# refresh-bio/fqsqueezer

Measured on AMD Instinct MI355X. Metric: Mbases/s compressed (DNA stream, SE sorted), higher is better.
Workload: dtype u64; 1 GPU; 1000000x150bp SE, G=7500000 (seed 2+rank), -om s -gs 8 -qm n -im n; workers_T=64, blocks=256, per_gpu=one independent file per GPU

## Files before the change

fqsqueezer_amd/codec.py:

```python
from __future__ import annotations

import ctypes as C
import os
from typing import List, Optional

import numpy as np

_PKG = os.path.dirname(os.path.abspath(__file__))
DEFAULT_LIB = os.path.join(_PKG, "libfqsx.so")

STAT_NAMES = ["gprobe", "gslot", "lprobe", "lslot", "gins", "gins_slot", "siv_words", "ctx_slots",
              "coded", "lins", "mail", "bases", "siv_saved", "dec_refetch"]


class FqsxError(RuntimeError):
    pass


def _load(path: str):
    if not os.path.exists(path):
        raise FqsxError(f"{path} not found: build it with `python -c 'import __graft_entry__ as g; g.build()'` "
                        "(hipcc --offload-arch=gfx950); there is no CPU fallback")
    try:
        import torch
    except ImportError:
        pass
    lib = C.CDLL(path)
    lib.fqsx_dna_create.restype = C.c_int
    lib.fqsx_dna_create.argtypes = [C.c_char_p, C.c_int, C.POINTER(C.c_void_p)]
    if hasattr(lib, "fqsx_dna_create_on_partition"):
        lib.fqsx_dna_create_on_partition.restype = C.c_int
        lib.fqsx_dna_create_on_partition.argtypes = [C.c_char_p, C.c_int, C.c_uint32, C.c_uint32, C.POINTER(C.c_void_p)]
    lib.fqsx_dna_destroy.argtypes = [C.c_void_p]
    lib.fqsx_dna_encode_block.restype = C.c_int
    lib.fqsx_dna_encode_block.argtypes = [C.c_void_p, C.c_void_p, C.c_void_p, C.c_uint32, C.c_uint32,
                                          C.POINTER(C.c_void_p), C.POINTER(C.c_uint64)]
    lib.fqsx_dna_encode_block_dev.restype = C.c_int
    lib.fqsx_dna_encode_block_dev.argtypes = [C.c_void_p, C.c_void_p, C.c_void_p, C.c_void_p, C.c_uint32, C.c_uint32,
                                              C.POINTER(C.c_void_p), C.POINTER(C.c_uint64)]
    lib.fqsx_dna_decode_block.restype = C.c_int
    lib.fqsx_dna_decode_block.argtypes = [C.c_void_p, C.POINTER(C.c_char_p), C.c_void_p, C.c_void_p, C.c_uint32, C.c_uint32, C.c_void_p]
    lib.fqsx_dna_stats.restype = C.c_int
    lib.fqsx_dna_stats.argtypes = [C.c_void_p, C.POINTER(C.c_uint64)]
    if hasattr(lib, "fqsx_dna_capacity"):
        lib.fqsx_dna_capacity.restype = C.c_int
# ... 352 lines not shown
```

fqsqueezer_amd/csrc/fqsx_api.hip:

```cpp
#include "fqsx_kernels.h"
#include "fqsx_qual.h"
#include "fqsx_qdec.h"
#include "../../include/fqsx.h"
#include "fqsx_vm.h"
#include "fqsx_rt.h"
#include <sys/resource.h>

#ifndef FQSX_EMU
#include <dlfcn.h>
#include <rccl/rccl.h>
#endif
#include <algorithm>
#include <cstdio>
#include <cstdlib>
#include <cstring>
#include <string>
#include <vector>

extern "C" const char *fqsx_last_error(void) { return g_err.c_str(); }
extern "C" const char *fqsx_version(void) {
#ifdef FQSX_EMU
  return "fqsx 0.1 (host emulation build - tests only)";
#else
  return "fqsx 0.1 (HIP gfx950)";
#endif
}

FQ_DEV bool phase_skip(const DevCfg &cfg) { return (cfg.err[0] | cfg.err[1]) != 0; }
#define FQSX_INS_THREADS 128
FQ_KERNEL128 void k_insert_phase(DevCfg cfg, u64 nb_slots, u64 ns_slots) {
  FQ_SHARED InsShared sm;
  if (phase_skip(cfg)) return;
#ifndef FQSX_EMU
  if (threadIdx.x == 0) { sm.pf_done = 0; sm.pf_on = blockDim.x > 64 ? 1u : 0u; }
  __syncthreads();
  if (FQ_WAVE_ID == 1) {
    if (FQ_BLOCK < 3 * cfg.T) insert_prefetch_body(cfg, &sm, FQ_BLOCK / 3, FQ_BLOCK % 3);
    return;
  }
#else
  sm.pf_done = 0; sm.pf_on = 0;
#endif
  if (FQ_BLOCK >= 3 * cfg.T) {
    const u64 stride = (u64)(FQ_NBLOCKS - 3 * cfg.T) * FQ_WAVE, first = (u64)(FQ_BLOCK - 3 * cfg.T) * FQ_WAVE + FQ_LANE;
    for (u64 i = first; i < nb_slots; i += stride) cfg.l_b.slots[i] = 0;
    for (u64 i = first; i < ns_slots; i += stride) cfg.l_s.slots[i] = 0;
    for (u64 i = first; i < 2ull * cfg.T; i += stride) cfg.l_s.filled[i] = 0;
    return;
  }
  insert_phase_body(cfg, &sm, FQ_BLOCK / 3, FQ_BLOCK % 3);
  if (cfg.sys_scope) fq_release_system();
}
FQ_KERNEL64 void k_compact_streams(DevCfg cfg, const u64 *lens, u8 *dst) {
  const u32 tid = FQ_BLOCK;
  u64 off = 0;
  for (u32 t = 0; t < tid; ++t) off += lens[t];
  const u64 n = lens[tid] <= cfg.out_cap ? lens[tid] : 0;
  const u8 *src = cfg.out + (u64)tid * cfg.out_cap;
  for (u64 i = FQ_LANE; i < n; i += FQ_WAVE) dst[off + i] = src[i];
}
FQ_KERNEL64 void k_compact_generic(const u8 *out, u64 out_cap, const u64 *lens, u8 *dst) {
  const u32 tid = FQ_BLOCK;
  u64 off = 0;
  for (u32 t = 0; t < tid; ++t) off += lens[t];
  const u64 n = lens[tid] <= out_cap ? lens[tid] : 0;
  const u8 *src = out + (u64)tid * out_cap;
  for (u64 i = FQ_LANE; i < n; i += FQ_WAVE) dst[off + i] = src[i];
}
FQ_KERNEL64 void k_clear_local(DevCfg cfg, u64 nb_slots, u64 ns_slots) {
  if (phase_skip(cfg)) return;
  const u64 stride = (u64)FQ_NBLOCKS * FQ_WAVE, first = (u64)FQ_BLOCK * FQ_WAVE + FQ_LANE;
  for (u64 i = first; i < nb_slots; i += stride) cfg.l_b.slots[i] = 0;
  for (u64 i = first; i < ns_slots; i += stride) cfg.l_s.slots[i] = 0;
  for (u64 i = first; i < 2ull * cfg.T; i += stride) cfg.l_s.filled[i] = 0;
}
FQ_KERNEL64 void k_finish_block(DevCfg cfg, u64 *lens , u64 *end ) {
  if (FQ_LANE == 0) {
    if (FQ_BLOCK == 0) { end[2 * cfg.T] = cfg.err[0]; end[2 * cfg.T + 1] = cfg.err[1]; }
    if (cfg.err[1]) return;
    finish_block_body(cfg, FQ_BLOCK);
    lens[FQ_BLOCK] = cfg.ws[FQ_BLOCK].out_len;
    end[FQ_BLOCK] = cfg.ws[FQ_BLOCK].out_len;
    end[cfg.T + FQ_BLOCK] = cfg.ctx_filled[FQ_BLOCK];
  }
// ... 436 lines not shown
  u32 cur_n_reads, cur_S, cur_gen;
  u64 cur_need_lb, cur_need_ls, cur_need_lpe;
  bool cur_decode;
  u32 shard_rank, shard_world = 1;
  u8 *d_vmap;
  u64 *d_xbuf;
  u64 xbuf_cap;
  u32 *d_cglob;
  u32 *d_colsum;
  u64 siv_before[2];
  fqsx_comm comm;
  bool comm_set, shard_apply_own;
  u64 *d_xrecv[3];
  u64 xrecv_cap[3];
  u64 *d_items, *d_gathered, *d_small;
  u64 items_cap, gathered_cap;
  std::vector<u32> h_cglob;
  u64 sh_phases, sh_collectives, sh_a2a_words, sh_gather_words;
  bool part;
  bool part_fallback;
  u64 vm_gran;
  fqsx_vm::FdMesh mesh;
  struct VmTab {
    u8 *va = nullptr;
    u64 va_bytes = 0, chunk_bytes = 0;
    std::vector<fqsx_vm::Handle> h;
    std::vector<u8> mapped;
    u64 own_bytes = 0;
    u32 own_mod = 0;
    bool live = false;
  } vm_s, vm_b, vm_pk, vm_pv, vm_siv;
  u32 *d_plog_n;
  u32 ins_threads;
  u64 vm_own_bytes;
};

namespace {

#define FQSX_PIN_BYTES (64u * 1024u)
int d2h_small_begin(fqsx_dna *c, const void *d, u64 bytes) { return d2h(c, c->h_pin, d, bytes); }
int d2h_small_end(fqsx_dna *c, void *h, u64 bytes) {
  DEVCHK(dev_sync(c));
  memcpy(h, c->h_pin, bytes);
  return FQSX_OK;
}

#define REHASH_GRID FQ_GRID(2048)

int collect_streams(DevCtx *c, u8 *&d_compact, u64 &compact_cap, u32 T, const u8 *d_out, u64 out_cap, const u64 *d_lens,
                    const std::vector<u64> &lens_host, std::vector<u8> &h_out, const u8 **streams, u64 *lens) {
  int rc;
  void *p = nullptr;
  u64 total = 0;
  for (u32 t = 0; t < T; ++t) total += lens_host[t];
  if (total > compact_cap) {
    dfree(c, d_compact);
    d_compact = nullptr; compact_cap = 0;
    if ((rc = dalloc(c, &p, total + total / 2 + 4096, false))) return rc;
    d_compact = (u8 *)p;
    compact_cap = total + total / 2 + 4096;
  }
  h_out.resize(total ? total : 1);
  if (total) {
    LAUNCH(c, 2, k_compact_generic, T, 64, d_out, out_cap, d_lens, d_compact);
    if ((rc = d2h_sync(c, h_out.data(), d_compact, total))) return rc;
  }
// ... 417 lines not shown
  }
  cfg.bases = d_bases;
  cfg.read_off = d_off;
  if (decode) {
    std::vector<u64> doff(T + 1, 0);
    for (u32 t = 0; t < T; ++t) doff[t + 1] = doff[t] + dec_lens[t];
    u64 max_len = 0;
    for (u32 i = 0; i < n_reads; ++i) max_len = std::max(max_len, h_off[i + 1] - h_off[i]);
    const u64 need_in = doff[T] + 64, need_out = h_off[n_reads] + 64, need_sc = max_len + 64;
    if (need_in > c->din_cap) {
      dfree(c, (void *)cfg.din);
      if ((rc = dalloc(c, &p, need_in + need_in / 4, false))) return rc;
      cfg.din = (const u8 *)p; c->din_cap = need_in + need_in / 4;
    }
    if (need_out > c->dout_cap) {
      dfree(c, cfg.dout);
      if ((rc = dalloc(c, &p, need_out + need_out / 4, false))) return rc;
      cfg.dout = (u8 *)p; c->dout_cap = need_out + need_out / 4;
    }
    if (need_sc > cfg.dcap) {
      dfree(c, cfg.dscratch);
      if ((rc = dalloc(c, &p, (u64)T * 2 * (need_sc + need_sc / 4), false))) return rc;
      cfg.dscratch = (u8 *)p; cfg.dcap = need_sc + need_sc / 4;
    }
    if (!cfg.din_off && (rc = dalloc(c, &p, ((u64)T + 1) * sizeof(u64), false))) return rc;
    if (!cfg.din_off) cfg.din_off = (const u64 *)p;
    std::vector<u8> flat(doff[T] ? doff[T] : 1);
    for (u32 t = 0; t < T; ++t) memcpy(flat.data() + doff[t], dec_streams[t], dec_lens[t]);
    if ((rc = h2d(c, (void *)cfg.din, flat.data(), doff[T]))) return rc;
    if ((rc = h2d(c, (void *)cfg.din_off, doff.data(), (T + 1) * sizeof(u64)))) return rc;
    DEVCHK(dev_sync(c));
  }

  c->cur_n_reads = n_reads; c->cur_S = (u32)S; c->cur_gen = generation;
  c->cur_need_lb = need_lb; c->cur_need_ls = need_ls; c->cur_need_lpe = need_lpe;
  c->cur_decode = decode;
  return FQSX_OK;
}

int clear_local_tables(fqsx_dna *c) {
  const u64 words = (c->cur_need_lb + c->cur_need_ls) * c->T;
  const u32 grid = (u32)std::min<u64>(2048, (words + 4095) / 4096 + 1);
  LAUNCH(c, 2, k_clear_local, grid, 64, c->cfg, c->cur_need_lb * c->T, c->cur_need_ls * c->T);
  return FQSX_OK;
}

int insert_and_clear(fqsx_dna *c) {
  const u64 words = (c->cur_need_lb + c->cur_need_ls) * c->T;
  const u32 cgrid = (u32)std::min<u64>(2048, (words + 4095) / 4096 + 1);
  LAUNCH(c, 1, k_insert_phase, 3 * c->T + cgrid, c->ins_threads, c->cfg, c->cur_need_lb * c->T, c->cur_need_ls * c->T);
  return FQSX_OK;
}
int grow_for_demand(fqsx_dna *c) {
  const u32 T = c->T;
  DevCfg &cfg = c->cfg;
  int rc;
  for (int which = 0; which < 2; ++which) {
    KTab &t = which ? cfg.g_b : cfg.g_s;
    u64 &cap = which ? c->gb_cap : c->gs_cap;
    u64 need = 0;
    for (u32 o = 0; o < T; ++o) need = std::max<u64>(need, (u64)c->h_demand[2 * T + 1 + which * T + o] + c->h_demand[which * T + o]);
    if (tab_over(c, need, cap) && (rc = grow_global(c, t, cap, tab_new_cap(c, need)))) return rc;
  }
  return FQSX_OK;
}
int pe_insert_and_clear(fqsx_dna *c);
int pe_clear_local(fqsx_dna *c);
int block_recover(fqsx_dna *c, u32 seg) {
  const u32 T = c->T;
  int rc;
  if ((rc = d2h_sync(c, c->h_demand.data(), c->d_demand, (4 * T + 1) * sizeof(u32)))) return rc;
  const u64 before = c->gs_cap + c->gb_cap + c->gpe_cap;
  if ((rc = grow_for_demand(c))) return rc;
  if ((rc = dzero(c, c->cfg.err + 1, sizeof(u32)))) return rc;
  if (c->paired) {
    if ((rc = dzero(c, c->cfg.pe_bkt_n, T * sizeof(u32)))) return rc;
    LAUNCH(c, 2, k_pe_demand, T, 64, c->cfg, c->d_demand + 4 * T + 1, 0u);
    std::vector<u32> dem(T), fil(T);
    if ((rc = d2h_sync(c, dem.data(), c->d_demand + 4 * T + 1, T * sizeof(u32)))) return rc;
    if ((rc = d2h_sync(c, fil.data(), c->cfg.g_pe.filled, T * sizeof(u32)))) return rc;
    u64 need = 0;
    for (u32 o = 0; o < T; ++o) need = std::max<u64>(need, (u64)fil[o] + dem[o]);
    if (need * 2 > c->gpe_cap && (rc = grow_gpe(c, pow2_at_least(need * 2 + 2)))) return rc;
  }
  if (c->gs_cap + c->gb_cap + c->gpe_cap == before) { g_err = "phase " + std::to_string(seg) + " posted for growth, but no table needs it"; return FQSX_E_DEVICE; }
  if (c->paired && (rc = pe_insert_and_clear(c))) return rc;
  return insert_and_clear(c);
}
int pe_clear_local(fqsx_dna *c) {
  const u32 T = c->T;
  DevCfg &cfg = c->cfg;
  int rc;
  if ((rc = dzero(c, cfg.l_pe.key, c->cur_need_lpe * T * sizeof(u64)))) return rc;
  if ((rc = dzero(c, cfg.l_pe.val, c->cur_need_lpe * T * sizeof(u64)))) return rc;
  return dzero(c, cfg.l_pe.filled, T * sizeof(u32));
}
int pe_insert_and_clear(fqsx_dna *c) {
  LAUNCH(c, 2, k_pe_insert, c->T, 64, c->cfg);
  return pe_clear_local(c);
}

int block_segment(fqsx_dna *c, u32 seg) {
  const u32 T = c->T, n_reads = c->cur_n_reads;
  const u64 S = c->cur_S, need_lpe = c->cur_need_lpe;
  const bool decode = c->cur_decode;
  DevCfg &cfg = c->cfg;
  int rc;
  {
    if ((rc = launch_segment(c, decode, n_reads, (u32)S, seg))) return rc;
    const u32 part_grid = T * (cfg.mail[0].n_tiles + cfg.mail[1].n_tiles + cfg.mail[2].n_tiles);
    LAUNCH(c, 2, k_part_count, part_grid, 64, cfg);
    LAUNCH(c, 2, k_part_scan, 3 * T, 64, cfg);
    if (!decode) {
      LAUNCH(c, 2, k_part_scatter, part_grid, 64, cfg, seg + 1, c->d_demand);
      if (c->paired) {
        const u32 bgrid = FQ_GRID((u32)std::min<u64>(1024, ((u64)T * cfg.pe_cap + 255) / 256));
        LAUNCH(c, 2, k_pe_bucket_count, bgrid, 256, cfg);
        LAUNCH(c, 2, k_pe_bucket_offsets, 1, 64, cfg, seg + 1);
        LAUNCH(c, 2, k_pe_bucket_scatter, bgrid, 256, cfg);
        LAUNCH(c, 2, k_pe_insert_buckets, T, 64, cfg);
        if ((rc = pe_clear_local(c))) return rc;
      }
      return insert_and_clear(c);
    }
    LAUNCH(c, 2, k_part_dstoff, 3, 64, cfg, c->d_demand, 0u);
    if ((rc = d2h_small_begin(c, c->d_demand, (4 * T + 1) * sizeof(u32)))) return rc;
    LAUNCH(c, 2, k_part_scatter, part_grid, 64, cfg, 0u, (u32 *)nullptr);
    if ((rc = d2h_small_end(c, c->h_demand.data(), (4 * T + 1) * sizeof(u32)))) return rc;
    if (c->h_demand[2 * T]) {
      g_err = "device error " + std::to_string(c->h_demand[2 * T]) + " in encode kernel";
      return FQSX_E_DEVICE;
    }
    if ((rc = grow_for_demand(c))) return rc;
    if (c->paired) {
      LAUNCH(c, 2, k_pe_demand, T, 64, cfg, c->d_demand, 0u);
      if ((rc = d2h_sync(c, c->h_demand.data(), c->d_demand, T * sizeof(u32)))) return rc;
      if ((rc = d2h_sync(c, c->h_filled.data(), cfg.g_pe.filled, T * sizeof(u32)))) return rc;
      u64 need = 0;
      for (u32 o = 0; o < T; ++o) need = std::max<u64>(need, (u64)c->h_filled[o] + c->h_demand[o]);
      if (need * 2 > c->gpe_cap && (rc = grow_gpe(c, pow2_at_least(need * 2 + 2)))) return rc;
      if ((rc = pe_insert_and_clear(c))) return rc;
    }
// ... 73 lines not shown
    seg = posted;
  }
  return rc;
}

int create_impl(fqsx_dna *c, const u8 *h) {
  const u32 T = c->T;
  DevCfg &cfg = c->cfg;
  memset(&cfg, 0, sizeof(cfg));
  cfg.T = T;
  cfg.mode = h[5];
  cfg.prefix = h[10]; cfg.pmer = h[11]; cfg.smer = h[12]; cfg.bmer = h[13];
  cfg.gp = make_geom(cfg.pmer); cfg.gs = make_geom(cfg.smer); cfg.gb = make_geom(cfg.bmer);
  cfg.pmer_mod_shift = 2 * cfg.pmer - 12;
  cfg.T_magic = ((1ull << 32) + T - 1) / T;
  cfg.T_pow2 = (T & (T - 1)) == 0 ? 1u : 0u;
  cfg.dbg = 0;
  if (const char *e = getenv("FQSX_PROTO_DEBUG")) cfg.dbg = (u32)strtoul(e, nullptr, 0);
  cfg.ps_nobytes_n = (2 * cfg.pmer + 7) / 8;
  int rc;
  void *p = nullptr;
  if ((rc = dalloc(c, &p, (1ull << (2 * cfg.pmer)) / 4, true))) return rc;
  cfg.siv = (u64 *)p;
  if ((rc = dalloc(c, &p, 2 * sizeof(u64), true))) return rc;
  cfg.siv_stats = (u64 *)p;
  if ((rc = dalloc(c, &p, ((1ull << (2 * cfg.pmer)) >> FQSX_SIV_BLK_LOG) * 4 * sizeof(u32), true))) return rc;
  cfg.siv_idx = (u32 *)p;
  c->tab_load_pct = 80; c->tab_after_pct = 62;
  if (const char *e = getenv("FQSX_TAB_LOAD_PCT")) c->tab_load_pct = (u32)std::min<u64>(85, std::max<u64>(20, strtoull(e, nullptr, 10)));
  c->tab_small_pct = 40;
  if (const char *e = getenv("FQSX_TAB_AFTER_PCT")) c->tab_small_pct = c->tab_after_pct = (u32)std::min<u64>(c->tab_load_pct - 5, std::max<u64>(10, strtoull(e, nullptr, 10)));
  cfg.tab_load_pct = c->tab_load_pct;
  c->ins_threads = (getenv("FQSX_INS_PREFETCH") && atoi(getenv("FQSX_INS_PREFETCH")) == 0) ? 64u : FQSX_INS_THREADS;
  if (const char *e = getenv("FQSX_WHATIF")) { u32 r = 0, u = 0; if (sscanf(e, "%u,%u", &r, &u) == 2) cfg.whatif = (r << 16) | (u & 0xffffu); }
  c->gs_cap = c->gb_cap = pow2_at_least(std::max<u64>(1024, (1ull << 22) / T));
  if (const char *e = getenv("FQSX_GTAB_INIT")) c->gs_cap = c->gb_cap = pow2_at_least(std::max<u64>(64, strtoull(e, nullptr, 10)));
  if ((rc = ktab_alloc(c, cfg.g_s, T, c->gs_cap, cfg.smer, 12, true))) return rc;
  if ((rc = ktab_alloc(c, cfg.g_b, T, c->gb_cap, cfg.bmer, 6, true))) return rc;
  cfg.g_s.two = cfg.g_b.two = 1;
  c->ls_cap = c->lb_cap = 1024;
  if ((rc = ktab_alloc(c, cfg.l_s, T, c->ls_cap, cfg.smer, 12, false))) return rc;
  if ((rc = ktab_alloc(c, cfg.l_b, T, c->lb_cap, cfg.bmer, 6, false))) return rc;
  if ((rc = dalloc(c, &p, 2 * (u64)T * sizeof(u32), true))) return rc;
  cfg.l_s.filled = (u32 *)p;
  cfg.l_b.filled = (u32 *)p + T;
  c->ctx_cap = 1u << 14;
  if ((rc = dalloc(c, &p, c->ctx_cap * T * sizeof(CtxSlot), true))) return rc;
  cfg.ctx = (CtxSlot *)p;
  cfg.ctx_cap_mask = c->ctx_cap - 1;
  if ((rc = dalloc(c, &p, T * sizeof(u32), true))) return rc;
  cfg.ctx_filled = (u32 *)p;
  {
    std::vector<u16> tpl(SM_OFF_BYTE, 0);
    auto fill = [&](u32 off, u32 entries, u32 stride, u32 n) {
      for (u32 e = 0; e < entries; ++e) {
        for (u32 i = 0; i < n; ++i) tpl[off + e * stride + i] = 1;
        tpl[off + e * stride + n] = (u16)n;
      }
    };
    fill(SM_OFF_FLAGS, 256, SM_FLAGS_N + 1, SM_FLAGS_N);
    fill(SM_OFF_NS, 32, SM_NS_N + 1, SM_NS_N);
    fill(SM_OFF_PSF, 65536, SM_PSF_N + 1, SM_PSF_N);
    fill(SM_OFF_PSNB, 65536, 6, cfg.ps_nobytes_n);
    fill(SM_OFF_NIB, 68, SM_NIB_N + 1, SM_NIB_N);
    tpl.resize(SM_TOTAL_U16, 0);
    fill(SM_OFF_MID, 1, SM_NIB_N + 1, SM_NIB_N);
// ... 706 lines not shown
int fqsx_rccl_comm_rebind(fqsx_comm *m, fqsx_dna *c) {
  if (!m || !m->ctx || !c) { g_err = "bad argument"; return FQSX_E_ARG; }
  ((RcclCtx *)m->ctx)->stream = c->stream;
  return FQSX_OK;
}
int fqsx_rccl_comm_info(fqsx_comm *m, uint32_t out[2]) {
  if (!m || !m->ctx || !out) { g_err = "bad argument"; return FQSX_E_ARG; }
  RcclCtx *x = (RcclCtx *)m->ctx;
  int n = 0, r = 0;
  if (g_rccl.CommCount(x->comm, &n) != ncclSuccess || g_rccl.CommUserRank(x->comm, &r) != ncclSuccess) { g_err = "ncclCommCount / ncclCommUserRank failed"; return FQSX_E_HIP; }
  out[0] = (u32)n; out[1] = (u32)r;
  return FQSX_OK;
}
void fqsx_rccl_comm_destroy(fqsx_comm *m) {
  if (!m || !m->ctx) return;
  RcclCtx *x = (RcclCtx *)m->ctx;
  if (g_rccl.CommDestroy && !x->aborted) (void)g_rccl.CommDestroy(x->comm);
  delete x;
  m->ctx = nullptr;
}
#else
static int no_rccl() { g_err = "the emulation build has no RCCL transport"; return FQSX_E_NO_DEVICE; }
int fqsx_rccl_unique_id(uint8_t *) { return no_rccl(); }
int fqsx_rccl_comm_create(fqsx_dna *, const uint8_t *, uint32_t, uint32_t, fqsx_comm *) { return no_rccl(); }
int fqsx_rccl_comm_rebind(fqsx_comm *, fqsx_dna *) { return no_rccl(); }
int fqsx_rccl_comm_info(fqsx_comm *, uint32_t *) { return no_rccl(); }
void fqsx_rccl_comm_destroy(fqsx_comm *) {}
#endif

int fqsx_dna_stats(fqsx_dna *c, uint64_t out[64]) {
  if (!c || !out) return FQSX_E_ARG;
  DEVCHK(dev_enter(c));
  LAUNCH(c, 2, k_gather_stats, 1, 64, c->cfg, c->d_lens + c->T);
  return d2h_sync(c, out, c->d_lens + c->T, 64 * sizeof(u64));
}

int fqsx_dna_capacity(fqsx_dna *c, uint64_t out[16]) {
  if (!c || !out) return FQSX_E_ARG;
  DEVCHK(dev_enter(c));
  const u32 T = c->T;
  std::vector<u32> f(T);
  int rc;
  for (int i = 0; i < 16; ++i) out[i] = 0;
  if ((rc = d2h_sync(c, f.data(), c->cfg.g_s.filled, T * sizeof(u32)))) return rc;
  for (u32 t = 0; t < T; ++t) out[0] += f[t];
  if ((rc = d2h_sync(c, f.data(), c->cfg.g_b.filled, T * sizeof(u32)))) return rc;
  for (u32 t = 0; t < T; ++t) out[1] += f[t];
  out[2] = c->gs_cap * T;
  out[3] = c->gb_cap * T;
  out[4] = (1ull << (2 * c->cfg.pmer)) / 4;
  out[5] = c->ctx_cap * T;
  if ((rc = d2h_sync(c, f.data(), c->cfg.ctx_filled, T * sizeof(u32)))) return rc;
  for (u32 t = 0; t < T; ++t) out[6] += f[t];
  out[7] = c->dev_bytes;
  out[8] = c->dev_bytes_peak;
  out[9] = c->n_growths;
  if (c->paired) {
    if ((rc = d2h_sync(c, f.data(), c->cfg.g_pe.filled, T * sizeof(u32)))) return rc;
    for (u32 t = 0; t < T; ++t) out[10] += f[t];
    out[11] = c->gpe_cap * T;
  }
  out[12] = sizeof(u64);
  out[13] = (c->vm_s.live ? c->vm_s.own_bytes : c->gs_cap * T * sizeof(u64)) + (c->vm_b.live ? c->vm_b.own_bytes : c->gb_cap * T * sizeof(u64));
  out[15] = c->vm_siv.live ? c->vm_siv.own_bytes : out[4];
  if (c->paired) out[14] = c->vm_pk.live ? c->vm_pk.own_bytes + c->vm_pv.own_bytes : c->gpe_cap * T * 2 * sizeof(u64);
  return FQSX_OK;
}
// ... 781 lines not shown
```

fqsqueezer_amd/csrc/fqsx_dev.h:

```cpp
#pragma once
#include "fqsx_layout.h"

#define FQSX_RR 6u
#define FQSX_SW 4u
#define FQSX_NSC 3u
#define FQSX_SCR FQSX_NSC
#define FQSX_RQ 256u
struct SpecBuf {
  u32 h_read, h_i0, h_n;
  u32 h_epoch;
  u32 h_pub;
  u32 h_fix_lane, h_fix_end;
  u32 h_pq_lo[2];
  u32 h_np, h_nlp;
  u64 h_ns, h_nls;
  u64 sp_sdir[6][FQSX_SPEC];
  u64 sp_src[6][FQSX_SPEC];
  u8 sp_scur[6][FQSX_SPEC];
  u64 sp_key[10][FQSX_SPEC];
  u8 sp_kind[FQSX_SPEC];
  u64 sp_cq[FQSX_SPEC];
  u8 sp_lvz[FQSX_SPEC];
  u8 sp_flag[FQSX_SPEC];
  u8 sp_rsym[FQSX_SPEC];
// ... 60 lines not shown
    u64 kdir[6], krc[6];
    u32 kcur[6];
    u64 s_let[4];
  } sc_req;
  u64 lev_tmp[10];
  u32 fr_idx[64], fr_c0[64], fr_thr[64], fr_vis[64];
  u64 fr_q1[64], fr_q2[64], fr_q3[64];
  u64 fr_same[64];
#ifdef FQSX_EMU
  u32 fr_f[64], fr_c[64], fr_t[64];
#endif
  u8 fr_lvl[64], fr_bad[64];
  u64 pq_key[2][FQSX_PQ];
  u64 ib_pos[64];
  u64 ib_hash[256];
  alignas(8) u32 qm_bits[4][256];
  u32 lq_target[2], lq_done[2], lq_quit;
  u64 cq_key[10][FQSX_CQ];
  u8 cq_kind[FQSX_CQ];
  u8 cq_rsym[FQSX_CQ];
  u32 cq_tail, cq_head, cq_done;
  u32 rq_f[FQSX_RQ], rq_c[FQSX_RQ], rq_t[FQSX_RQ];
  u64 rq_m[FQSX_RQ];
  u32 rq_tail, rq_head, rq_done;
  u32 wg_stop;
};
#ifndef FQSX_EMU
static_assert(sizeof(WgShared) <= 160u * 1024u, "WgShared must fit the 160 KB of LDS of a gfx950 CU");
#endif
struct InsShared {
  u32 mt[4][624];
  u32 mt_idx[4];
  u32 pf_done, pf_on;
  u64 ib_pos[64];
  u64 ib_hash[256];
  u64 bk_key[64];
  u64 pe_bk[3][64];
};
struct EncArgs {
  DevCfg cfg;
  u32 n_reads, S, seg, pad;
};
#ifndef FQSX_EMU
__shared__ WgShared fq_wg_lds;
FQ_DEV WgShared *fq_wg() { return &fq_wg_lds; }
typedef const __attribute__((address_space(4))) EncArgs *FqArgsP;
FQ_DEV FqArgsP fq_kernarg() { return (FqArgsP)__builtin_amdgcn_kernarg_segment_ptr(); }
FQ_DEV const EncArgs *fq_args(FqArgsP a) {
  const unsigned long v = (unsigned long)a;
  const u32 lo = __builtin_amdgcn_readfirstlane((u32)v), hi = __builtin_amdgcn_readfirstlane((u32)(v >> 32));
  return (const EncArgs *)(FqArgsP)(((unsigned long)hi << 32) | lo);
}
#else
typedef const EncArgs *FqArgsP;
FQ_DEV WgShared *fq_wg() { static thread_local WgShared s; return &s; }
FQ_DEV const EncArgs *fq_args(FqArgsP a) { return a; }
#endif
enum { SX_VALID = 1, SX_LB = 2, SX_S = 4, SX_LS = 8, SX_UNC = 16 ,
       SX_HITS = SX_LB | SX_S | SX_LS | SX_UNC };
enum { SCQ_FROM_HEAD = 1 , SCQ_REVERSED = 2  };
enum { SK_NONE = 0, SK_RANK = 1, SK_LETTER = 2, SK_RANK_PENDING = 3, SK_LETTER_PENDING = 4, SK_RAW = 5, SK_KIND_MASK = 7,
       SK_RESET = 8  };
enum { PV_B = 1, PV_S = 2, PV_P = 4, PV_PHID = 8, PV_PCAND = 16 };

struct C4 { u32 c[4]; };
struct Kmer { u64 dir, rc; u32 cur; };
// ... 518 lines not shown
FQ_DEV void batch_hit_mask(Wk &w, u32 n, u64 mask[4]) {
  WgShared *sm = w.sm;
  mask[0] = mask[1] = mask[2] = mask[3] = 0;
#if FQ_WAVE > 1
  for (u32 r = 0; r * 64 < n; ++r) {
    u32 q = r * 64 + FQ_LANE;
    bool hit = q < n && (sm->bk_res[q][0] | sm->bk_res[q][1] | sm->bk_res[q][2] | sm->bk_res[q][3]) != 0;
    mask[r] = wave_ballot(hit);
  }
#else
  for (u32 q = 0; q < n; ++q)
    if (sm->bk_res[q][0] | sm->bk_res[q][1] | sm->bk_res[q][2] | sm->bk_res[q][3]) mask[q >> 6] |= 1ull << (q & 63);
#endif
}
FQ_DEV void batch_count(Wk &w, const KTab &t, u32 n) {
  WgShared *sm = w.sm;
  u64 ns = 0;
  FQ_SYNC();
  for (u32 i = FQ_LANE; i < n; i += FQ_WAVE) {
    u64 key = sm->bk_key[i];
    sm->bk_res[i][0] = tab_count(t, sb_owner(w.cfg, key), key, ns);
  }
  FQ_SYNC();
  w.st[ST_GPROBE] += n;
  w.st[ST_GSLOT] += wave_sum64(ns);
}

template <class SM>
FQ_DEV void insert_batch(const DevCfg &cfg, SM *sm, const KTab &t, u32 sub, const u64 *keys, u32 n, u32 rng, const Cinc &ci,
                         u64 &nslots, u32 &err);
template <class SM>
FQ_DEV void insert_batch_k(const DevCfg &cfg, SM *sm, const KTab &t, u32 sub, u64 mykey, u32 n, u32 rng, const Cinc &ci,
                           u64 &nslots, u32 &err);
template <class SM, bool EXT_PF = false>
FQ_DEV void insert_keys(const DevCfg &cfg, SM *sm, const KTab &t, u32 sub, const u64 *keys, u32 n, u32 rng, const Cinc &ci,
                        u64 &nslots, u32 &err) {
#if FQ_WAVE > 1
  if constexpr (EXT_PF) {
    u64 nextk = FQ_LANE < n ? keys[FQ_LANE] : 0;
    for (u32 o = 0; o < n && !err; o += FQ_WAVE) {
      const u64 k = nextk;
      if (o + FQ_WAVE + FQ_LANE < n) nextk = keys[o + FQ_WAVE + FQ_LANE];
      insert_batch_k(cfg, sm, t, sub, k, n - o < FQ_WAVE ? n - o : FQ_WAVE, rng, ci, nslots, err);
      lds_store_rel(&sm->pf_done, o / FQ_WAVE + 1);
    }
    return;
  }
  const u64 *s = t.slots + (u64)sub * t.stride;
  u64 nextk = FQ_LANE < n ? keys[FQ_LANE] : 0;
  for (u32 o = 0; o < n && !err; o += FQ_WAVE) {
    const u64 k = nextk;
    u64 touch = 0;
    if (o + FQ_WAVE + FQ_LANE < n) {
      nextk = keys[o + FQ_WAVE + FQ_LANE];
      const TabHome th = tab_home(t, nextk >> (64 - 2 * t.k));
      touch = touch_load(&s[(u64)th.a * FQSX_BKT]) ^ touch_load(&s[(u64)th.b * FQSX_BKT]);
    }
    insert_batch_k(cfg, sm, t, sub, k, n - o < FQ_WAVE ? n - o : FQ_WAVE, rng, ci, nslots, err);
    keep_live(touch);
  }
#else
  for (u32 j = 0; j < n && !err; ++j) insert_batch(cfg, sm, t, sub, keys + j, 1, rng, ci, nslots, err);
#endif
}
FQ_DEV u32 lq_done_now(Wk &w, u32 qi) { return w.lqh ? lds_load_acq(&w.sm->lq_done[qi]) : w.la[qi ? MAIL_S : MAIL_B]; }
FQ_DEV void lq_publish(Wk &w, bool force = false) {
// ... 3424 lines not shown
  TM_TRACE_VAL(cfg, tid, launch, 12, w.tm[TM_RRWAIT]); TM_TRACE_VAL(cfg, tid, launch, 13, w.tm[TM_SPEC]);
  TM_TRACE_VAL(cfg, tid, launch, 14, w.tm[CN_GENERIC]); TM_TRACE_VAL(cfg, tid, launch, 15, w.tm[TM_LQ]);
#ifdef FQSX_TIMING
  {
    const u32 xs[16] = {TM_SLOW, TM_SPRE, TM_ROUGH, TM_FINDC, TM_POST, TM_KEYS, TM_READ_HEAD, TM_CQWAIT, TX_QMM, TX_QRUN, TX_PROLOG, TX_CHUNKQ, TX_FLUSH, TM_TOTAL, TX_G_EARLY, TX_OWNSPEC};
    for (u32 x = 0; x < 16; ++x) TM_TRACE_VAL(cfg, tid, launch, 16 + x, w.tm[xs[x]]);
  }
#endif
  if (!piped) {
    for (u32 i = 0; i < ST_N; ++i) ws->stat[i] += w.st[i];
    for (u32 i = 0; i < FQSX_TM_SLOTS && i < 48; ++i) ws->stat[16 + i] += w.tm[i];
  } else if (FQ_LANE == 0) {
    for (u32 i = 0; i < ST_N; ++i) if (w.st[i]) atomic_add64(&ws->stat[i], w.st[i]);
#ifdef FQSX_TIMING
    for (u32 i = 0; i < FQSX_TM_SLOTS && i < 48; ++i) if (w.tm[i]) atomic_add64(&ws->stat[16 + i], w.tm[i]);
#endif
  }
  FQ_SYNC();
  mt_copy((u64 *)&ws->mt[0][0], (const u64 *)&sm->mt[0][0]);
  for (u32 g = FQ_LANE; g < 4; g += FQ_WAVE) ws->mt_idx[g] = sm->mt_idx[g];
  for (u32 k = 0; k < 3; ++k) cfg.mail[k].n[tid] = w.mn[k];
  if (paired) cfg.pe_n[tid] = w.pe_n;
  if (w.err) *cfg.err = w.err;
}

template <class SM>
FQ_DEV void insert_batch(const DevCfg &cfg, SM *sm, const KTab &t, u32 tid, const u64 *keys, u32 n, u32 rng, const Cinc &ci,
                         u64 &nslots, u32 &err) {
  insert_batch_k(cfg, sm, t, tid, FQ_LANE < n ? keys[FQ_LANE] : 0, n, rng, ci, nslots, err);
}
template <class SM>
FQ_DEV void insert_batch_k(const DevCfg &cfg, SM *sm, const KTab &t, u32 tid, u64 mykey, u32 n, u32 rng, const Cinc &ci,
                           u64 &nslots, u32 &err) {
  (void)cfg;
#ifdef FQSX_TIMING
  u64 ib_t[4] = {0, 0, 0, 0}, ib_rounds = 0;
#define IB_MARK(i) do { const u64 now_ = fq_clock(); ib_t[i] += now_ - ib_c; ib_c = now_; } while (0)
  u64 ib_c = fq_clock();
#else
#define IB_MARK(i) ((void)0)
#endif
  u64 *s = t.slots + (u64)tid * t.stride;
  const u64 cm = (1ull << t.cbits) - 1ull;
  const u32 lane = FQ_LANE;
  const u64 v = lane < n ? mykey >> (64 - 2 * t.k) : 0;
  u32 filled = t.filled[tid];
  for (u32 done = 0; done < n;) {
    u64 pos = 0, item = 0;
    bool act = lane >= done && lane < n, found = false;
    if (act) {
      const TabLoc L = t.two ? tab_locate(t, s, v) : tab_locate1(t, s, v);
      pos = L.pos; item = L.item; nslots += L.ns;
      found = item != 0;
    }
    IB_MARK(0);
    u32 lim = n;
#if FQ_WAVE > 1
    FQ_SYNC();
    sm->ib_pos[lane] = act ? pos : ~0ull;
    for (u32 i = lane; i < 256; i += FQ_WAVE) sm->ib_hash[i] = 0;
    FQ_SYNC();
    const u32 hb = (((u32)pos ^ (u32)(pos >> 32)) * 0x9E3779B1u) >> 24;
    if (act) lds_or64(&sm->ib_hash[hb], 1ull << lane);
    FQ_SYNC();
    bool clash = false;
    if (act) {
      u64 cand = sm->ib_hash[hb] & ((1ull << lane) - 1ull);
      while (cand && !clash) {
        const u32 j = ctz64(cand);
        cand &= cand - 1ull;
        clash = sm->ib_pos[j] == pos;
      }
    }
    const u64 cl = wave_ballot(clash);
    if (cl) lim = ctz64(cl);
    act = act && lane < lim;
#else
    lim = done + 1;
#endif
    IB_MARK(1);
    const u32 n_new = popc64(wave_ballot(act && !found));
    if ((u64)(filled + n_new) * 10 >= t.nb * FQSX_BKT * 9) { err = FQSX_ERR_GTAB_FULL; return; }
    const u32 cnt = (u32)(item & cm);
    const bool draw = act && found && cnt > ci.thr && cnt < ci.maxv;
    const u64 dm = wave_ballot(draw);
    u32 r = 0;
    if (dm) {
      const u32 my = popc64(dm & ((1ull << lane) - 1ull)), total = popc64(dm);
      u32 idx = sm->mt_idx[rng];
      const u32 avail = idx >= 624 ? 0 : 624 - idx;
      if (draw && my < avail) r = mt_temper(sm->mt[rng][idx + my]);
      if (total > avail) {
        mt_twist(sm->mt[rng]);
        if (draw && my >= avail) r = mt_temper(sm->mt[rng][my - avail]);
        idx = total - avail;
      } else
        idx += total;
      FQ_SYNC();
      if (lane == 0) sm->mt_idx[rng] = idx;
      FQ_SYNC();
    }
    if (act) {
      if (!found) s[pos] = (v << t.cbits) | 1ull;
      else if (cnt <= ci.thr) { if (cnt < (u32)cm) s[pos] = item + 1; }
      else if (draw && (r % (ci.mult * (cnt - ci.thr)) == 0)) s[pos] = item + 1;
    }
    filled += n_new;
    done = lim;
    if (lane == 0 && done >= n) t.filled[tid] = filled;
    IB_MARK(2);
    FQ_SYNC_MEM();
    IB_MARK(3);
#ifdef FQSX_TIMING
    ++ib_rounds;
#endif
  }
#ifdef FQSX_TIMING
  if (rng < 2 && lane == 0) {
    for (u32 i = 0; i < 4; ++i) atomic_add64(&cfg.ws[tid].stat[16 + 40 + i], ib_t[i]);
    atomic_add64(&cfg.ws[tid].stat[16 + 44], ib_rounds);
// ... 64 lines not shown
    (void)cnt; (void)ld;
    if (e < hi) lds_or64(&gm[d], 1ull << FQ_LANE);
    FQ_SYNC();
    const u64 mine = e < hi ? gm[d] : 0;
    const u32 rank = popc64(mine & ((1ull << FQ_LANE) - 1ull));
    const u32 later = (mine >> FQ_LANE) >> 1 ? 1u : 0u;
    u32 cur = e < hi ? cursor[d] : 0;
    FQ_SYNC();
    if (e < hi) {
      m.sorted[cur + rank] = x;
      if (later == 0) { cursor[d] = cur + rank + 1; gm[d] = 0; }
    }
    FQ_SYNC();
#else
    ld[FQ_LANE] = d;
    FQ_SYNC();
    u32 rank = 0, later = 0;
    for (u32 q = 0; q < cnt; ++q) {
      u32 dq = ld[q];
      rank += (q < FQ_LANE && dq == d) ? 1u : 0u;
      later += (q > FQ_LANE && dq == d) ? 1u : 0u;
    }
    u32 cur = e < hi ? cursor[d] : 0;
    FQ_SYNC();
    if (e < hi) {
      m.sorted[cur + rank] = x;
      if (later == 0) cursor[d] = cur + rank + 1;
    }
    FQ_SYNC();
#endif
  }
}

FQ_DEV void siv_idx_move(const DevCfg &cfg, u64 idx, u32 from, u32 to) {
  u32 *e = cfg.siv_idx + 4 * (idx >> FQSX_SIV_BLK_LOG);
#ifndef FQSX_EMU
  if (from) atomicSub(&e[from], 1u);
  atomicAdd(&e[to], 1u);
#else
  if (from) e[from] -= 1;
  e[to] += 1;
#endif
}
#ifndef FQSX_PF_AHEAD
#define FQSX_PF_AHEAD 4
#endif
#if FQ_WAVE > 1
template <class SM>
FQ_DEV void insert_prefetch_body(const DevCfg &cfg, SM *sm, u32 tid, u32 kind) {
  if (kind == MAIL_P) return;
  const Mail &m = cfg.mail[kind];
  const u32 lo = m.dst_off[tid], hi = m.dst_off[tid + 1], n = hi - lo;
  const KTab &t = kind == MAIL_S ? cfg.g_s : cfg.g_b;
  const u64 *s = t.slots + (u64)tid * t.stride, *keys = m.sorted + lo;
  u64 acc = 0;
  for (u32 o = 0; o < n; o += FQ_WAVE) {
    u32 spins = 0;
    while ((i32)(o / FQ_WAVE - lds_load_acq(&sm->pf_done)) > (i32)FQSX_PF_AHEAD) {
      fq_sleep();
      if (++spins > (1u << 18)) { keep_live(acc); return; }
    }
    if (o + FQ_LANE < n) {
      const TabHome th = tab_home(t, keys[o + FQ_LANE] >> (64 - 2 * t.k));
      acc ^= touch_load(&s[(u64)th.a * FQSX_BKT]) ^ touch_load(&s[(u64)th.b * FQSX_BKT]);
    }
  }
  keep_live(acc);
}
#endif
template <class SM>
FQ_DEV void insert_phase_body(const DevCfg &cfg, SM *sm, u32 tid, u32 kind) {
  WState *ws = cfg.ws + tid;
  const Mail &m = cfg.mail[kind];
  const u32 lo = m.dst_off[tid], hi = m.dst_off[tid + 1];
  if (kind == MAIL_P) {
    u64 nf = 0, nu = 0;
    for (u32 e = lo + FQ_LANE; e < hi; e += FQ_WAVE) {
      u64 idx = m.sorted[e];
      u64 *wp = cfg.siv + (idx >> 5);
      u32 sh = 2 * (u32)(idx & 31);
      u64 old = *wp;
      for (;;) {
        u64 f = (old >> sh) & 3;
        if (f == 3) break;
        u64 seen = atomic_cas64(wp, old, old + (1ull << sh));
        if (seen == old) {
          nf += f == 0;
          siv_idx_move(cfg, idx, (u32)f, (u32)f + 1);
          if (cfg.siv_part) {
#ifndef FQSX_EMU
            const u32 at = atomicAdd(cfg.p_log_n, 1u);
#else
            const u32 at = (*cfg.p_log_n)++;
#endif
            cfg.p_log[at] = (idx << 4) | (f << 2) | (f + 1);
          }
          break;
        }
        old = seen;
      }
      ++nu;
    }
    nf = wave_sum64(nf);
    nu = wave_sum64(nu);
    if (FQ_LANE == 0) {
#ifndef FQSX_EMU
      atomicAdd((unsigned long long *)&cfg.siv_stats[1], (unsigned long long)nf);
      atomicAdd((unsigned long long *)&cfg.siv_stats[0], (unsigned long long)(nu + ws->hidden_updates));
#else
      cfg.siv_stats[1] += nf;
      cfg.siv_stats[0] += nu + ws->hidden_updates;
#endif
      ws->hidden_updates = 0;
      ws->stat[ST_SIV_WORDS] += hi - lo;
    }
    return;
  }
  const KTab &t = kind == MAIL_S ? cfg.g_s : cfg.g_b;
  const u32 rng = kind == MAIL_S ? RNG_S : RNG_B;
  const Cinc ci = kind == MAIL_S ? CINC_S : CINC_B;
  u32 err = 0;
  u64 n_slots = 0;
  FQ_SYNC();
  for (u32 i = FQ_LANE; i < 624; i += FQ_WAVE) sm->mt[rng][i] = ws->mt[rng][i];
  if (FQ_LANE == 0) sm->mt_idx[rng] = ws->mt_idx[rng];
  FQ_SYNC();
  if (sm->pf_on) insert_keys<SM, true>(cfg, sm, t, tid, m.sorted + lo, hi - lo, rng, ci, n_slots, err);
  else insert_keys(cfg, sm, t, tid, m.sorted + lo, hi - lo, rng, ci, n_slots, err);
  FQ_SYNC();
  for (u32 i = FQ_LANE; i < 624; i += FQ_WAVE) ws->mt[rng][i] = sm->mt[rng][i];
  n_slots = wave_sum64(n_slots);
  if (FQ_LANE == 0) {
    ws->mt_idx[rng] = sm->mt_idx[rng];
#ifndef FQSX_EMU
    atomicAdd((unsigned long long *)&ws->stat[ST_GINS], (unsigned long long)(hi - lo));
    atomicAdd((unsigned long long *)&ws->stat[ST_GINS_SLOT], (unsigned long long)n_slots);
#else
    ws->stat[ST_GINS] += hi - lo;
    ws->stat[ST_GINS_SLOT] += n_slots;
#endif
  }
  if (err) *cfg.err = err;
}

FQ_DEV void finish_block_body(const DevCfg &cfg, u32 tid) {
  WState *ws = cfg.ws + tid;
  u64 low = ws->rc_low, len = ws->out_len;
  u8 *out = cfg.out + (u64)tid * cfg.out_cap;
  for (int i = 0; i < 8; ++i) {
    if (len < cfg.out_cap) out[len] = (u8)(low >> 56); else *cfg.err = FQSX_ERR_OUT_OVERFLOW;
    ++len;
    low <<= 8;
  }
  ws->rc_low = low;
  ws->out_len = len;
}
```

Baseline: 109.8 Mbases/s.

## Fuse mail partition, demand check and global insert into one phase-tail kernel

Adds a k_phase_tail kernel that replaces the per-phase sequence of partition count/scan/scatter and insert launches with a single launch. Each owner workgroup gathers its mailbox keys directly into LDS using multiple waves, writes demand and the growth flag itself, then inserts with a companion prefetch wave. It also loads the Mersenne-Twister state lazily, only when a random draw is actually needed. The goal is to cut kernel-launch and global sort/scatter traffic per phase, at the cost of a done-stamp recovery protocol, more complex control flow, and a key-count limit above which the old split path is used.

Measured after the change: 110.2 Mbases/s (median of 6 runs). Within noise of the previous version (+0.4%).

```diff
diff --git a/fqsqueezer_amd/codec.py b/fqsqueezer_amd/codec.py
--- a/fqsqueezer_amd/codec.py
+++ b/fqsqueezer_amd/codec.py
@@ -10,7 +10,7 @@
 DEFAULT_LIB = os.path.join(_PKG, "libfqsx.so")
 
 STAT_NAMES = ["gprobe", "gslot", "lprobe", "lslot", "gins", "gins_slot", "siv_words", "ctx_slots",
-              "coded", "lins", "mail", "bases", "siv_saved", "dec_refetch"]
+              "coded", "lins", "mail", "bases", "siv_saved", "dec_refetch", "phases_fused", "phases_split"]
 
 
 class FqsxError(RuntimeError):
diff --git a/fqsqueezer_amd/csrc/fqsx_api.hip b/fqsqueezer_amd/csrc/fqsx_api.hip
--- a/fqsqueezer_amd/csrc/fqsx_api.hip
+++ b/fqsqueezer_amd/csrc/fqsx_api.hip
@@ -50,6 +50,102 @@
   }
   insert_phase_body(cfg, &sm, FQ_BLOCK / 3, FQ_BLOCK % 3);
   if (cfg.sys_scope) fq_release_system();
+}
+#define FQSX_TAIL_THREADS (64u * FQSX_TAIL_WAVES)
+#define FQSX_TAIL_TOTAL_MAX 65536u
+FQ_KERNEL512 void k_phase_tail(DevCfg cfg, u64 nb_slots, u64 ns_slots, u32 seg1, u32 *demand , u32 *done ,
+                               u32 stamp, u32 stage, u32 recover) {
+  FQ_SHARED TailShared sm;
+  const u32 T = cfg.T, wave = FQ_WAVE_ID;
+#ifndef FQSX_EMU
+  const u32 nw = blockDim.x >> 6, tix = threadIdx.x;
+#else
+  const u32 nw = 1, tix = 0;
+#endif
+  const bool owner_wg = FQ_BLOCK < 3 * T;
+  const u32 d = FQ_BLOCK / 3, kind = FQ_BLOCK % 3;
+  u32 e0 = 0, e1 = 0, dn = 0, fl = 0;
+  if (tix == 0) {
+    e0 = cfg.err[0]; e1 = cfg.err[1];
+    if (owner_wg) {
+      dn = done[kind * T + d];
+      if (kind != MAIL_P) fl = (kind == MAIL_S ? cfg.g_s : cfg.g_b).filled[d];
+    }
+  }
+  if (owner_wg) {
+    for (u32 i = tix; i < T; i += nw * FQ_WAVE) sm.n_src[i] = cfg.mail[kind].n[i];
+    for (u32 i = tix; i < 256; i += nw * FQ_WAVE) sm.vm[i] = cfg.vmap[i];
+  }
+  if (tix == 0) {
+    bool go = !(e0 || (e1 && e1 != seg1));
+    if (go && owner_wg && recover && dn == stamp) go = false;
+    sm.go = go ? 1u : 0u;
+    sm.filled = fl;
+    sm.ins.pf_done = 0; sm.ins.pf_on = 0; sm.ins.mt_have = 0;
+  }
+  FQ_WG_BARRIER();
+  if (!sm.go) return;
+  if (!owner_wg) {
+    if (wave) return;
+    const u64 stride = (u64)(FQ_NBLOCKS - 3 * T) * FQ_WAVE, first = (u64)(FQ_BLOCK - 3 * T) * FQ_WAVE + FQ_LANE;
+    for (u64 i = first; i < nb_slots; i += stride) cfg.l_b.slots[i] = 0;
+    for (u64 i = first; i < ns_slots; i += stride) cfg.l_s.slots[i] = 0;
+    for (u64 i = first; i < 2ull * T; i += stride) cfg.l_s.filled[i] = 0;
+    return;
+  }
+  u32 tot = 0;
+  bool whole = true;
+  TailCur cur = {0, 0, 0};
+  if (nw > 1) {
+    const u32 pw = stage / nw;
+    TailCur mine = {wave * T / nw, 0, 0};
+    const u32 c = tail_gather(cfg, kind, d, sm.n_src, sm.vm, (wave + 1) * T / nw, mine, 0, pw, sm.part + wave * pw, true);
+    if (FQ_LANE == 0) sm.cnt[wave] = c;
+    FQ_WG_BARRIER();
+    u32 off = 0;
+    for (u32 w = 0; w < nw; ++w) {
+      const u32 cw = sm.cnt[w];
+      if (w < wave) off += cw;
+      tot += cw;
+      whole = whole && cw <= pw;
+    }
+    if (whole)
+      for (u32 i = FQ_LANE; i < c; i += FQ_WAVE) sm.keys[off + i] = sm.part[wave * pw + i];
+  } else
+    tot = tail_gather(cfg, kind, d, sm.n_src, sm.vm, T, cur, 0, stage, sm.keys, true);
+  if (tix == 0) {
+    u32 post = 0;
+    if (!recover) {
+      if (kind == MAIL_P) {
+        if (d == 0) demand[2 * T] = cfg.err[0];
+      } else {
+        const KTab &t = kind == MAIL_S ? cfg.g_s : cfg.g_b;
+        const u32 o = (kind == MAIL_S ? 0 : T) + d, filled = sm.filled;
+        demand[o] = tot;
+        demand[2 * T + 1 + o] = filled;
+        if (((u64)filled + tot) * 100 > t.nb * FQSX_BKT * cfg.tab_load_pct) { cfg.err[1] = seg1; post = 1; }
+      }
+    }
+    sm.post = post;
+    sm.ins.pf_on = (nw > 1 && whole && !post) ? 1u : 0u;
+  }
+  FQ_WG_BARRIER();
+  if (sm.post) return;
+#if FQ_WAVE > 1
+  if (wave == 1 && whole) insert_prefetch_keys(cfg, &sm.ins, d, kind, sm.keys, tot);
+#endif
+  if (wave) return;
+  bool staged = nw == 1 || whole;
+  u32 base = 0;
+  do {
+    if (!staged) tail_gather(cfg, kind, d, sm.n_src, sm.vm, T, cur, base, stage, sm.keys, false);
+    staged = false;
+    insert_group(cfg, &sm.ins, d, kind, sm.keys, tot - base < stage ? tot - base : stage);
+    base += stage;
+  } while (base < tot);
+  insert_group_end(cfg, &sm.ins, d, kind);
+  lds_store_rel(&sm.ins.pf_done, 0x7fffffffu);
+  if (FQ_LANE == 0) done[kind * T + d] = stamp;
 }
 FQ_KERNEL64 void k_compact_streams(DevCfg cfg, const u64 *lens, u8 *dst) {
   const u32 tid = FQ_BLOCK;
@@ -552,6 +648,12 @@
   } vm_s, vm_b, vm_pk, vm_pv, vm_siv;
   u32 *d_plog_n;
   u32 ins_threads;
+  bool tail_on;
+  bool cur_fused;
+  u32 tail_stage;
+  u32 *d_tail_done;
+  u32 tail_stamp, cur_stamp0;
+  u64 n_tail_fused, n_tail_split;
   u64 vm_own_bytes;
 };
 
@@ -1035,6 +1137,15 @@
     DEVCHK(dev_sync(c));
   }
 
+  c->cur_fused = c->tail_on && !decode && !c->paired && (u64)T * std::max(mail_entries[0], mail_entries[2]) <= FQSX_TAIL_TOTAL_MAX;
+  if (c->cur_fused) {
+    if (c->tail_stamp > 0xffffffffu - (u32)(S + 2)) {
+      if ((rc = dzero(c, c->d_tail_done, 3 * (u64)T * sizeof(u32)))) return rc;
+      c->tail_stamp = 0;
+    }
+    c->cur_stamp0 = c->tail_stamp;
+    c->tail_stamp += (u32)S + 1;
+  }
   c->cur_n_reads = n_reads; c->cur_S = (u32)S; c->cur_gen = generation;
   c->cur_need_lb = need_lb; c->cur_need_ls = need_ls; c->cur_need_lpe = need_lpe;
   c->cur_decode = decode;
@@ -1052,6 +1163,13 @@
   const u64 words = (c->cur_need_lb + c->cur_need_ls) * c->T;
   const u32 cgrid = (u32)std::min<u64>(2048, (words + 4095) / 4096 + 1);
   LAUNCH(c, 1, k_insert_phase, 3 * c->T + cgrid, c->ins_threads, c->cfg, c->cur_need_lb * c->T, c->cur_need_ls * c->T);
+  return FQSX_OK;
+}
+int phase_tail(fqsx_dna *c, u32 seg, bool recover) {
+  const u64 words = (c->cur_need_lb + c->cur_need_ls) * c->T;
+  const u32 cgrid = recover ? 0u : (u32)std::min<u64>(2048, (words + 4095) / 4096 + 1);
+  LAUNCH(c, 1, k_phase_tail, 3 * c->T + cgrid, c->ins_threads == 64 ? 64u : FQSX_TAIL_THREADS, c->cfg, c->cur_need_lb * c->T,
+         c->cur_need_ls * c->T, seg + 1, c->d_demand, c->d_tail_done, c->cur_stamp0 + seg + 1, c->tail_stage, recover ? 1u : 0u);
   return FQSX_OK;
 }
 int grow_for_demand(fqsx_dna *c) {
@@ -1088,7 +1206,7 @@
   }
   if (c->gs_cap + c->gb_cap + c->gpe_cap == before) { g_err = "phase " + std::to_string(seg) + " posted for growth, but no table needs it"; return FQSX_E_DEVICE; }
   if (c->paired && (rc = pe_insert_and_clear(c))) return rc;
-  return insert_and_clear(c);
+  return c->cur_fused ? phase_tail(c, seg, true) : insert_and_clear(c);
 }
 int pe_clear_local(fqsx_dna *c) {
   const u32 T = c->T;
@@ -1111,6 +1229,8 @@
   int rc;
   {
     if ((rc = launch_segment(c, decode, n_reads, (u32)S, seg))) return rc;
+    if (c->cur_fused) { c->n_tail_fused += 1; return phase_tail(c, seg, false); }
+    c->n_tail_split += 1;
     const u32 part_grid = T * (cfg.mail[0].n_tiles + cfg.mail[1].n_tiles + cfg.mail[2].n_tiles);
     LAUNCH(c, 2, k_part_count, part_grid, 64, cfg);
     LAUNCH(c, 2, k_part_scan, 3 * T, 64, cfg);
@@ -1250,6 +1370,12 @@
   if (const char *e = getenv("FQSX_TAB_AFTER_PCT")) c->tab_small_pct = c->tab_after_pct = (u32)std::min<u64>(c->tab_load_pct - 5, std::max<u64>(10, strtoull(e, nullptr, 10)));
   cfg.tab_load_pct = c->tab_load_pct;
   c->ins_threads = (getenv("FQSX_INS_PREFETCH") && atoi(getenv("FQSX_INS_PREFETCH")) == 0) ? 64u : FQSX_INS_THREADS;
+  c->tail_on = !(getenv("FQSX_PHASE_FUSED") && atoi(getenv("FQSX_PHASE_FUSED")) == 0);
+  c->tail_stage = FQSX_TAIL_STAGE;
+  if (const char *e = getenv("FQSX_TAIL_STAGE")) c->tail_stage = (u32)std::min<u64>(FQSX_TAIL_STAGE, std::max<u64>(64, strtoull(e, nullptr, 10) / 64 * 64));
+  if ((rc = dalloc(c, &p, 3 * (u64)T * sizeof(u32), true))) return rc;
+  c->d_tail_done = (u32 *)p;
+  c->tail_stamp = 0; c->n_tail_fused = c->n_tail_split = 0;
   if (const char *e = getenv("FQSX_WHATIF")) { u32 r = 0, u = 0; if (sscanf(e, "%u,%u", &r, &u) == 2) cfg.whatif = (r << 16) | (u & 0xffffu); }
   c->gs_cap = c->gb_cap = pow2_at_least(std::max<u64>(1024, (1ull << 22) / T));
   if (const char *e = getenv("FQSX_GTAB_INIT")) c->gs_cap = c->gb_cap = pow2_at_least(std::max<u64>(64, strtoull(e, nullptr, 10)));
@@ -2022,7 +2148,10 @@
   if (!c || !out) return FQSX_E_ARG;
   DEVCHK(dev_enter(c));
   LAUNCH(c, 2, k_gather_stats, 1, 64, c->cfg, c->d_lens + c->T);
-  return d2h_sync(c, out, c->d_lens + c->T, 64 * sizeof(u64));
+  DEVCHK(d2h_sync(c, out, c->d_lens + c->T, 64 * sizeof(u64)));
+  out[14] = c->n_tail_fused;
+  out[15] = c->n_tail_split;
+  return FQSX_OK;
 }
 
 int fqsx_dna_capacity(fqsx_dna *c, uint64_t out[16]) {
diff --git a/fqsqueezer_amd/csrc/fqsx_dev.h b/fqsqueezer_amd/csrc/fqsx_dev.h
--- a/fqsqueezer_amd/csrc/fqsx_dev.h
+++ b/fqsqueezer_amd/csrc/fqsx_dev.h
@@ -116,6 +116,7 @@
   u32 mt[4][624];
   u32 mt_idx[4];
   u32 pf_done, pf_on;
+  u32 mt_have, pad_;
   u64 ib_pos[64];
   u64 ib_hash[256];
   u64 bk_key[64];
@@ -700,6 +701,16 @@
 template <class SM>
 FQ_DEV void insert_batch_k(const DevCfg &cfg, SM *sm, const KTab &t, u32 sub, u64 mykey, u32 n, u32 rng, const Cinc &ci,
                            u64 &nslots, u32 &err);
+template <class SM>
+FQ_DEV void mt_need(SM *, const DevCfg &, u32, u32) {}
+FQ_DEV void mt_need(InsShared *sm, const DevCfg &cfg, u32 tid, u32 rng) {
+  if ((sm->mt_have >> rng) & 1u) return;
+  const WState *ws = cfg.ws + tid;
+  FQ_SYNC();
+  for (u32 i = FQ_LANE; i < 624; i += FQ_WAVE) sm->mt[rng][i] = ws->mt[rng][i];
+  if (FQ_LANE == 0) { sm->mt_idx[rng] = ws->mt_idx[rng]; sm->mt_have |= 1u << rng; }
+  FQ_SYNC();
+}
 template <class SM, bool EXT_PF = false>
 FQ_DEV void insert_keys(const DevCfg &cfg, SM *sm, const KTab &t, u32 sub, const u64 *keys, u32 n, u32 rng, const Cinc &ci,
                         u64 &nslots, u32 &err) {
@@ -4190,7 +4201,6 @@
 template <class SM>
 FQ_DEV void insert_batch_k(const DevCfg &cfg, SM *sm, const KTab &t, u32 tid, u64 mykey, u32 n, u32 rng, const Cinc &ci,
                            u64 &nslots, u32 &err) {
-  (void)cfg;
 #ifdef FQSX_TIMING
   u64 ib_t[4] = {0, 0, 0, 0}, ib_rounds = 0;
 #define IB_MARK(i) do { const u64 now_ = fq_clock(); ib_t[i] += now_ - ib_c; ib_c = now_; } while (0)
@@ -4244,6 +4254,7 @@
     const u64 dm = wave_ballot(draw);
     u32 r = 0;
     if (dm) {
+      mt_need(sm, cfg, tid, rng);
       const u32 my = popc64(dm & ((1ull << lane) - 1ull)), total = popc64(dm);
       u32 idx = sm->mt_idx[rng];
       const u32 avail = idx >= 624 ? 0 : 624 - idx;
@@ -4374,6 +4385,71 @@
   }
 }
 
+#define FQSX_TAIL_STAGE 2048u
+#define FQSX_TAIL_WAVES 8u
+struct TailShared {
+  InsShared ins;
+  u64 keys[FQSX_TAIL_STAGE];
+  u64 part[FQSX_TAIL_STAGE];
+  u32 cnt[FQSX_TAIL_WAVES];
+  u32 n_src[256];
+  u8 vm[256];
+  u32 go, post, filled;
+};
+#define FQSX_TAIL_UNROLL 14
+struct TailCur { u32 s, e, run; };
+FQ_DEV u32 tail_gather(const DevCfg &cfg, u32 kind, u32 d, const u32 *n_src , const u8 *vm , u32 s_hi,
+                       TailCur &cur, u32 r_lo, u32 cap, u64 *out , bool all) {
+  const Mail &m = cfg.mail[kind];
+  const u32 per = 2 * FQ_WAVE;
+  const u64 below = (1ull << FQ_LANE) - 1ull;
+  u32 s = cur.s, e = cur.e, run = cur.run;
+  bool have_next = false;
+  while (s < s_hi && n_src[s] <= e) { ++s; e = 0; }
+  while (s < s_hi) {
+    const TailCur here = {s, e, run};
+    u64 x0[FQSX_TAIL_UNROLL], x1[FQSX_TAIL_UNROLL];
+    u32 left[FQSX_TAIL_UNROLL];
+#pragma unroll
+    for (u32 u = 0; u < FQSX_TAIL_UNROLL; ++u) {
+      left[u] = 0; x0[u] = x1[u] = 0;
+      if (s < s_hi) {
+        const u32 n = n_src[s], at = e + 2 * FQ_LANE;
+        if (at < n) {
+          const u64 *p = m.list + (u64)s * m.cap + at;
+#ifndef FQSX_EMU
+          const ulonglong2 v = *(const ulonglong2 *)p;
+          x0[u] = v.x; x1[u] = v.y;
+#else
+          x0[u] = p[0]; x1[u] = p[1];
+#endif
+          left[u] = n - at;
+        }
+        e += per;
+        if (e >= n) { e = 0; ++s; while (s < s_hi && n_src[s] == 0) ++s; }
+      }
+    }
+#pragma unroll
+    for (u32 u = 0; u < FQSX_TAIL_UNROLL; ++u) {
+      const bool m0 = left[u] > 0 && vm[mail_owner(cfg, kind, x0[u])] == d;
+      const bool m1 = left[u] > 1 && vm[mail_owner(cfg, kind, x1[u])] == d;
+      const u64 b0 = wave_ballot(m0), b1 = wave_ballot(m1);
+      const u32 r0 = run + popc64(b0 & below) + popc64(b1 & below) - r_lo, r1 = r0 + (m0 ? 1u : 0u);
+      if (m0 && r0 < cap) out[r0] = x0[u];
+      if (m1 && r1 < cap) out[r1] = x1[u];
+      run += popc64(b0) + popc64(b1);
+    }
+    if (!have_next && run >= r_lo + cap) {
+      cur = here;
+      have_next = true;
+      if (!all) break;
+    }
+  }
+  if (!have_next) { cur.s = s_hi; cur.e = 0; cur.run = run; }
+  FQ_SYNC();
+  return run;
+}
+
 FQ_DEV void siv_idx_move(const DevCfg &cfg, u64 idx, u32 from, u32 to) {
   u32 *e = cfg.siv_idx + 4 * (idx >> FQSX_SIV_BLK_LOG);
 #ifndef FQSX_EMU
@@ -4389,12 +4465,10 @@
 #endif
 #if FQ_WAVE > 1
 template <class SM>
-FQ_DEV void insert_prefetch_body(const DevCfg &cfg, SM *sm, u32 tid, u32 kind) {
+FQ_DEV void insert_prefetch_keys(const DevCfg &cfg, SM *sm, u32 tid, u32 kind, const u64 *keys, u32 n) {
   if (kind == MAIL_P) return;
-  const Mail &m = cfg.mail[kind];
-  const u32 lo = m.dst_off[tid], hi = m.dst_off[tid + 1], n = hi - lo;
   const KTab &t = kind == MAIL_S ? cfg.g_s : cfg.g_b;
-  const u64 *s = t.slots + (u64)tid * t.stride, *keys = m.sorted + lo;
+  const u64 *s = t.slots + (u64)tid * t.stride;
   u64 acc = 0;
   for (u32 o = 0; o < n; o += FQ_WAVE) {
     u32 spins = 0;
@@ -4409,16 +4483,20 @@
   }
   keep_live(acc);
 }
-#endif
 template <class SM>
-FQ_DEV void insert_phase_body(const DevCfg &cfg, SM *sm, u32 tid, u32 kind) {
-  WState *ws = cfg.ws + tid;
+FQ_DEV void insert_prefetch_body(const DevCfg &cfg, SM *sm, u32 tid, u32 kind) {
   const Mail &m = cfg.mail[kind];
   const u32 lo = m.dst_off[tid], hi = m.dst_off[tid + 1];
+  insert_prefetch_keys(cfg, sm, tid, kind, m.sorted + lo, hi - lo);
+}
+#endif
+template <class SM>
+FQ_DEV void insert_group(const DevCfg &cfg, SM *sm, u32 tid, u32 kind, const u64 *keys, u32 n) {
+  WState *ws = cfg.ws + tid;
   if (kind == MAIL_P) {
     u64 nf = 0, nu = 0;
-    for (u32 e = lo + FQ_LANE; e < hi; e += FQ_WAVE) {
-      u64 idx = m.sorted[e];
+    for (u32 e = FQ_LANE; e < n; e += FQ_WAVE) {
+      u64 idx = keys[e];
       u64 *wp = cfg.siv + (idx >> 5);
       u32 sh = 2 * (u32)(idx & 31);
       u64 old = *wp;
@@ -4454,7 +4532,7 @@
       cfg.siv_stats[0] += nu + ws->hidden_updates;
 #endif
       ws->hidden_updates = 0;
-      ws->stat[ST_SIV_WORDS] += hi - lo;
+      ws->stat[ST_SIV_WORDS] += n;
     }
     return;
   }
@@ -4463,26 +4541,38 @@
   const Cinc ci = kind == MAIL_S ? CINC_S : CINC_B;
   u32 err = 0;
   u64 n_slots = 0;
-  FQ_SYNC();
-  for (u32 i = FQ_LANE; i < 624; i += FQ_WAVE) sm->mt[rng][i] = ws->mt[rng][i];
-  if (FQ_LANE == 0) sm->mt_idx[rng] = ws->mt_idx[rng];
-  FQ_SYNC();
-  if (sm->pf_on) insert_keys<SM, true>(cfg, sm, t, tid, m.sorted + lo, hi - lo, rng, ci, n_slots, err);
-  else insert_keys(cfg, sm, t, tid, m.sorted + lo, hi - lo, rng, ci, n_slots, err);
-  FQ_SYNC();
-  for (u32 i = FQ_LANE; i < 624; i += FQ_WAVE) ws->mt[rng][i] = sm->mt[rng][i];
+  if (sm->pf_on) insert_keys<SM, true>(cfg, sm, t, tid, keys, n, rng, ci, n_slots, err);
+  else insert_keys(cfg, sm, t, tid, keys, n, rng, ci, n_slots, err);
   n_slots = wave_sum64(n_slots);
   if (FQ_LANE == 0) {
-    ws->mt_idx[rng] = sm->mt_idx[rng];
 #ifndef FQSX_EMU
-    atomicAdd((unsigned long long *)&ws->stat[ST_GINS], (unsigned long long)(hi - lo));
+    atomicAdd((unsigned long long *)&ws->stat[ST_GINS], (unsigned long long)n);
     atomicAdd((unsigned long long *)&ws->stat[ST_GINS_SLOT], (unsigned long long)n_slots);
 #else
-    ws->stat[ST_GINS] += hi - lo;
+    ws->stat[ST_GINS] += n;
     ws->stat[ST_GINS_SLOT] += n_slots;
 #endif
   }
   if (err) *cfg.err = err;
+}
+template <class SM>
+FQ_DEV void insert_group_end(const DevCfg &cfg, SM *sm, u32 tid, u32 kind) {
+  if (kind == MAIL_P) return;
+  WState *ws = cfg.ws + tid;
+  const u32 rng = kind == MAIL_S ? RNG_S : RNG_B;
+  FQ_SYNC();
+  if (!((sm->mt_have >> rng) & 1u)) return;
+  for (u32 i = FQ_LANE; i < 624; i += FQ_WAVE) ws->mt[rng][i] = sm->mt[rng][i];
+  if (FQ_LANE == 0) ws->mt_idx[rng] = sm->mt_idx[rng];
+}
+template <class SM>
+FQ_DEV void insert_phase_body(const DevCfg &cfg, SM *sm, u32 tid, u32 kind) {
+  const Mail &m = cfg.mail[kind];
+  const u32 lo = m.dst_off[tid], hi = m.dst_off[tid + 1];
+  if (FQ_LANE == 0) sm->mt_have = 0;
+  FQ_SYNC();
+  insert_group(cfg, sm, tid, kind, m.sorted + lo, hi - lo);
+  insert_group_end(cfg, sm, tid, kind);
 }
 
 FQ_DEV void finish_block_body(const DevCfg &cfg, u32 tid) {
```
